# maybeLx/MVSFormerPlusPlus

Hardware: AMD Instinct MI355X
Metric: ref-views/sec at 1152x1536 N=5 D=192 4-stage; achieved HBM GB/s vs peak (higher is better)
Workload: dtype fp16 operands/storage, fp32 accumulate (every stage; 1-2 fp16 MFMA terms)

## Files before the change

mvsformerplusplus_amd/csrc/vis_kernels.hip:

```cpp
#include "mvs_common.h"

namespace mvs {

typedef __bf16 vs_bf16x8 __attribute__((ext_vector_type(8)));
typedef __bf16 vs_bf16x4 __attribute__((ext_vector_type(4)));

constexpr int VS_TW = 60;
constexpr int VS_P = 64;
constexpr int VS_RING = 4;
constexpr int VS_SH_MAX = 64;
constexpr int VS_EP = VS_P + 2;
constexpr int VS_ENT_BYTES = (VS_SH_MAX + 6) * VS_EP * 4;
constexpr int VS_F16_PLANE_SHIFT = 0;
template <bool F16>
struct VsL {
    static constexpr int POSB = F16 ? 16 : 32;
    static constexpr int PLANE = ((VS_RING * VS_P + 2) * POSB + 255) / 256 * 256 + (F16 ? VS_F16_PLANE_SHIFT : 16);
    static constexpr int LAYER = 2 * PLANE;
    static constexpr int LDS = 2 * LAYER + VS_ENT_BYTES;
};
typedef _Float16 vs_f16x8 __attribute__((ext_vector_type(8)));
typedef _Float16 vs_f16x4 __attribute__((ext_vector_type(4)));

#ifndef MVS_OPAQUE_VEC
#define MVS_OPAQUE_VEC "v"
#endif

__device__ __forceinline__ vs_f16x4 vs_mask4(vs_f16x4 h, bool in) {
    typedef unsigned vs_u32x2 __attribute__((ext_vector_type(2)));
    vs_u32x2 u = __builtin_bit_cast(vs_u32x2, h);
    u[0] = in ? u[0] : 0u;
    u[1] = in ? u[1] : 0u;
    return __builtin_bit_cast(vs_f16x4, u);
}

__device__ __forceinline__ vs_f16x4 vs_cvt4(const float* v) {
    typedef float vs_f32x4 __attribute__((ext_vector_type(4)));
    return __builtin_convertvector((vs_f32x4){v[0], v[1], v[2], v[3]}, vs_f16x4);
}

__device__ __forceinline__ void vs_split4(const float* v, vs_bf16x4& hi, vs_bf16x4& lo) {
#pragma unroll
    for (int j = 0; j < 4; ++j) {
        const __bf16 h = (__bf16)v[j];
        hi[j] = h;
        lo[j] = (__bf16)(v[j] - (float)h);
    }
}

template <int SLOT0, int POSB>
__device__ __forceinline__ int vs_step_off(int laneoff, int tapsel, int t) {
    const int tapA = 2 * t, tapB = 2 * t + 1 < 9 ? 2 * t + 1 : 8;
    const int offA = (((SLOT0 + tapA / 3) & (VS_RING - 1)) * VS_P + tapA % 3) * POSB;
    const int offB = (((SLOT0 + tapB / 3) & (VS_RING - 1)) * VS_P + tapB % 3) * POSB;
    return laneoff + (tapsel ? offB : offA);
}

struct VsOperand { vs_bf16x8 h, l; };
template <bool F16>
__device__ __forceinline__ VsOperand vs_load(const char* p) {
    VsOperand o;
    o.h = *reinterpret_cast<const vs_bf16x8*>(p);
    if constexpr (!F16) o.l = *reinterpret_cast<const vs_bf16x8*>(p + 16);
    else o.l = o.h;
    return o;
}

template <bool F16>
__device__ __forceinline__ f32x4 vs_mfma_lo(const vs_bf16x8& wl, const VsOperand& x, f32x4 a) {
    if constexpr (F16) return __builtin_amdgcn_mfma_f32_16x16x32_f16(__builtin_bit_cast(vs_f16x8, wl), __builtin_bit_cast(vs_f16x8, x.h), a, 0, 0, 0);
    else return __builtin_amdgcn_mfma_f32_16x16x32_bf16(wl, x.h, a, 0, 0, 0);
}
template <bool F16>
__device__ __forceinline__ f32x4 vs_mfma_hi(const vs_bf16x8& wh, const VsOperand& x, f32x4 a) {
    if constexpr (F16) return __builtin_amdgcn_mfma_f32_16x16x32_f16(__builtin_bit_cast(vs_f16x8, wh), __builtin_bit_cast(vs_f16x8, x.h), a, 0, 0, 0);
    else return __builtin_amdgcn_mfma_f32_16x16x32_bf16(wh, x.h, a, 0, 0, 0);
}

template <int SLOT0, bool F16, bool ONE = false>
__device__ __forceinline__ f32x4 vs_layer_row(const char* lds_layer, int laneoff, int tapsel, const vs_bf16x8* wh, const vs_bf16x8* wl, f32x4 init) {
    constexpr int POSB = VsL<F16>::POSB;
    f32x4 a0 = {0.0f, 0.0f, 0.0f, 0.0f}, a1 = a0, a2 = init;
    VsOperand cur = vs_load<F16>(lds_layer + vs_step_off<SLOT0, POSB>(laneoff, tapsel, 0));
#pragma unroll
    for (int t = 0; t < 5; ++t) {
        VsOperand nxt = cur;
        if (t < 4) nxt = vs_load<F16>(lds_layer + vs_step_off<SLOT0, POSB>(laneoff, tapsel, t + 1));
        __builtin_amdgcn_sched_barrier(0);
        if constexpr (!ONE) a0 = vs_mfma_lo<F16>(wl[t], cur, a0);
        if constexpr (!F16) a1 = __builtin_amdgcn_mfma_f32_16x16x32_bf16(wh[t], cur.l, a1, 0, 0, 0);
        a2 = vs_mfma_hi<F16>(wh[t], cur, a2);
        cur = nxt;
    }
    return a0 + a1 + a2;
}

template <int SLOT2, int SLOT3, bool F16, bool ONE = false>
__device__ __forceinline__ void vs_two_layer_rows(const char* lds1, const char* lds2, int laneoff, int tapsel, const vs_bf16x8* w2h,
                                                  const vs_bf16x8* w2l, const vs_bf16x8* w3h, const vs_bf16x8* w3l, f32x4& out2, f32x4& out3) {
    constexpr int POSB = VsL<F16>::POSB;
    f32x4 a = out2, c = out3;
    VsOperand cb = vs_load<F16>(lds1 + vs_step_off<SLOT2, POSB>(laneoff, tapsel, 0));
    VsOperand cc = vs_load<F16>(lds2 + vs_step_off<SLOT3, POSB>(laneoff, tapsel, 0));
#pragma unroll
    for (int t = 0; t < 5; ++t) {
        VsOperand nb = cb, nc = cc;
        if (t < 4) {
            nb = vs_load<F16>(lds1 + vs_step_off<SLOT2, POSB>(laneoff, tapsel, t + 1));
            nc = vs_load<F16>(lds2 + vs_step_off<SLOT3, POSB>(laneoff, tapsel, t + 1));
        }
        __builtin_amdgcn_sched_barrier(0);
        if constexpr (!ONE) {
            a = vs_mfma_lo<F16>(w2l[t], cb, a);
            c = vs_mfma_lo<F16>(w3l[t], cc, c);
        }
        if constexpr (!F16) {
            a = __builtin_amdgcn_mfma_f32_16x16x32_bf16(w2h[t], cb.l, a, 0, 0, 0);
            c = __builtin_amdgcn_mfma_f32_16x16x32_bf16(w3h[t], cc.l, c, 0, 0, 0);
        }
        a = vs_mfma_hi<F16>(w2h[t], cb, a);
        c = vs_mfma_hi<F16>(w3h[t], cc, c);
        cb = nb;
        cc = nc;
    }
    out2 = a;
    out3 = c;
}

template <int V> struct VsInt { static constexpr int value = V; };

template <bool F16, bool ONE = false>
__global__ __launch_bounds__(256) void vis_cnn_kernel(const float* __restrict__ ent, const float* __restrict__ w1 ,
                                                      const float* __restrict__ b1, const void* __restrict__ wp2, const float* __restrict__ b2,
                                                      const void* __restrict__ wp3, const float* __restrict__ b3, const float* __restrict__ w4,
                                                      const float* __restrict__ b4, float* __restrict__ vis, int H, int W, int SH) {
    HIP_DYNAMIC_SHARED(float4, lds4)
    char* lds1 = reinterpret_cast<char*>(lds4);
    constexpr int VS_POSB = VsL<F16>::POSB, VS_PLANE = VsL<F16>::PLANE, VS_LAYER = VsL<F16>::LAYER;
    char* lds2 = lds1 + VS_LAYER;
    const int tid = (int)threadIdx.x, lane = tid & 63;
    const int wave = __builtin_amdgcn_readfirstlane(tid >> 6);
    const int li = lane & 15, g = lane >> 4;
    const int x0 = (int)blockIdx.x * VS_TW, r0 = (int)blockIdx.y * SH;
    const int r1 = r0 + SH < H ? r0 + SH : H;
    const float* e = ent + (size_t)blockIdx.z * H * W;
    float* vo = vis + (size_t)blockIdx.z * H * W;

    vs_bf16x8 w2h[5], w2l[5], w3h[5], w3l[5];
    {
        const vs_bf16x8* q2 = reinterpret_cast<const vs_bf16x8*>(wp2) + lane;
        const vs_bf16x8* q3 = reinterpret_cast<const vs_bf16x8*>(wp3) + lane;
#pragma unroll
        for (int t = 0; t < 5; ++t) {
            w2h[t] = q2[(t * 2) * 64]; w2l[t] = q2[(t * 2 + 1) * 64];
            w3h[t] = q3[(t * 2) * 64]; w3l[t] = q3[(t * 2 + 1) * 64];
#ifndef MVS_NO_OPAQUE_VEC
            if constexpr (ONE) asm volatile("" : "+" MVS_OPAQUE_VEC(w2h[t]), "+" MVS_OPAQUE_VEC(w3h[t]));
            else asm volatile("" : "+" MVS_OPAQUE_VEC(w2h[t]), "+" MVS_OPAQUE_VEC(w2l[t]), "+" MVS_OPAQUE_VEC(w3h[t]), "+" MVS_OPAQUE_VEC(w3l[t]));
#endif
        }
    }
    constexpr bool L1MFMA = F16 && ONE;
    vs_f16x8 w1a = {0, 0, 0, 0, 0, 0, 0, 0};
    f32x4 b1q = {0.0f, 0.0f, 0.0f, 0.0f};
    if constexpr (L1MFMA) {
        const int kh = g < 3 ? g : 0;
#pragma unroll
        for (int kw = 0; kw < 3; ++kw) {
            const _Float16 wv = g < 3 ? (_Float16)w1[(kh * 3 + kw) * 16 + li] : (_Float16)0.0f;
            w1a[kw] = wv;
            w1a[3 + kw] = wv;
        }
#pragma unroll
        for (int r = 0; r < 4; ++r) b1q[r] = b1[4 * g + r];
    }
    float w1s[9][4], b1s[4];
#pragma unroll
    for (int t = 0; t < 9; ++t)
#pragma unroll
        for (int r = 0; r < 4; ++r) w1s[t][r] = w1[t * 16 + 4 * wave + r];
#pragma unroll
    for (int r = 0; r < 4; ++r) b1s[r] = b1[4 * wave + r];
    float b2v[4], b3v[4], w4v[4];
#pragma unroll
    for (int r = 0; r < 4; ++r) {
        b2v[r] = b2[4 * g + r];
        b3v[r] = g < 2 ? b3[4 * g + r] : 0.0f;
        w4v[r] = g < 2 ? w4[4 * g + r] : 0.0f;
    }
    const float bias4 = b4[0];

    const int xa = x0 - 2 + lane;
    const int i0 = r0 - 2, i1 = r1 + 4;
    float* ent_s = reinterpret_cast<float*>(lds1 + 2 * VS_LAYER);
    {
        const int nrow = r1 - r0 + 6;
        for (int idx = tid; idx < nrow * VS_EP; idx += 256) {
            const int rr = idx / VS_EP, cc = idx - rr * VS_EP;
            const int yy = r0 - 3 + rr, xx = x0 - 3 + cc;
            ent_s[idx] = (yy >= 0 && yy < H && xx >= 0 && xx < W) ? e[(size_t)yy * W + xx] : 0.0f;
        }
    }
    __syncthreads();
    const int colmaskA = xa >= 0 && xa < W;
    const int wrA = (wave >> 1) * VS_PLANE + lane * VS_POSB + (wave & 1) * 8;
    const int laneoff = (g & 1) * VS_PLANE + (16 * wave + li) * VS_POSB;
    const int wrB = (g >> 1) * VS_PLANE + (16 * wave + li) * VS_POSB + (g & 1) * 8;
    const int tapsel = g >> 1;
    const int c2 = 16 * wave + li;
    const int xb = x0 - 1 + c2, xc = x0 + c2;

    auto iteration = [&](auto phase, auto steady, int i) __attribute__((always_inline)) {
        constexpr int PH = decltype(phase)::value;
        constexpr bool STEADY = decltype(steady)::value != 0;
        if constexpr (L1MFMA) {
            if (STEADY || i <= r1 + 1) {
                const float* ep = ent_s + (i - 1 + (g < 3 ? g : 2) - (r0 - 3)) * VS_EP + c2;
                const float e0 = ep[0], e1 = ep[1], e2 = ep[2];
                typedef float vs_f32x2 __attribute__((ext_vector_type(2)));
                typedef _Float16 vs_f16x2 __attribute__((ext_vector_type(2)));
                typedef unsigned vs_u32x4 __attribute__((ext_vector_type(4)));
                const unsigned p0 = __builtin_bit_cast(unsigned, __builtin_convertvector((vs_f32x2){e0, e1}, vs_f16x2));
                const float l0 = MVS_FMA_MIX_LO(p0, -1.0f, e0), l1 = MVS_FMA_MIX_HI(p0, -1.0f, e1);
                const unsigned p1 = __builtin_bit_cast(unsigned, __builtin_convertvector((vs_f32x2){e2, l0}, vs_f16x2));
                const float l2 = MVS_FMA_MIX_LO(p1, -1.0f, e2);
                const unsigned p2 = __builtin_bit_cast(unsigned, __builtin_convertvector((vs_f32x2){l1, l2}, vs_f16x2));
                const vs_f16x8 bop = __builtin_bit_cast(vs_f16x8, (vs_u32x4){p0, p1, p2, 0u});
                const f32x4 r1v = __builtin_amdgcn_mfma_f32_16x16x32_f16(w1a, bop, b1q, 0, 0, 0);
                const int xa1 = x0 - 2 + c2;
                const bool in = xa1 >= 0 && xa1 < W && i >= 0 && i < H;
                float a[4];
#pragma unroll
                for (int r = 0; r < 4; ++r) a[r] = fmaxf(r1v[r], 0.0f);
                *reinterpret_cast<vs_f16x4*>(lds1 + wrB + PH * (VS_P * VS_POSB)) = vs_mask4(vs_cvt4(a), in);
            }
        } else if (STEADY || i <= r1 + 1) {
            float er[3][3];
            const float* ep = ent_s + (i - 1 - (r0 - 3)) * VS_EP + lane;
#pragma unroll
            for (int kh = 0; kh < 3; ++kh)
#pragma unroll
                for (int kw = 0; kw < 3; ++kw) er[kh][kw] = ep[kh * VS_EP + kw];
            typedef float f32x2 __attribute__((ext_vector_type(2)));
            f32x2 a01 = {b1s[0], b1s[1]}, a23 = {b1s[2], b1s[3]};
#pragma unroll
            for (int kh = 0; kh < 3; ++kh)
#pragma unroll
                for (int kw = 0; kw < 3; ++kw) {
                    const f32x2 ev = {er[kh][kw], er[kh][kw]};
                    a01 = __builtin_elementwise_fma(ev, (f32x2){w1s[kh * 3 + kw][0], w1s[kh * 3 + kw][1]}, a01);
                    a23 = __builtin_elementwise_fma(ev, (f32x2){w1s[kh * 3 + kw][2], w1s[kh * 3 + kw][3]}, a23);
                }
            float a[4] = {a01[0], a01[1], a23[0], a23[1]};
            const bool in = colmaskA && i >= 0 && i < H;
#pragma unroll
            for (int r = 0; r < 4; ++r) a[r] = F16 ? fmaxf(a[r], 0.0f) : (in ? fmaxf(a[r], 0.0f) : 0.0f);
            char* p = lds1 + wrA + PH * (VS_P * VS_POSB);
            if constexpr (F16) {
                *reinterpret_cast<vs_f16x4*>(p) = vs_mask4(vs_cvt4(a), in);
            } else {
                vs_bf16x4 hi, lo;
                vs_split4(a, hi, lo);
                *reinterpret_cast<vs_bf16x4*>(p) = hi;
                *reinterpret_cast<vs_bf16x4*>(p + 16) = lo;
            }
        }
        const int yb = i - 2, yc = i - 4;
        const bool doB = STEADY || (yb >= r0 - 1 && yb <= r1), doC = STEADY || yc >= r0;
        constexpr int S2 = (PH + 1) & 3, S3 = (PH + 3) & 3;
        f32x4 acc2 = {b2v[0], b2v[1], b2v[2], b2v[3]}, acc3 = {b3v[0], b3v[1], b3v[2], b3v[3]};
        if (STEADY || (doB && doC)) vs_two_layer_rows<S2, S3, F16, ONE>(lds1, lds2, laneoff, tapsel, w2h, w2l, w3h, w3l, acc2, acc3);
        else if (doB) acc2 = vs_layer_row<S2, F16, ONE>(lds1, laneoff, tapsel, w2h, w2l, acc2);
        else if (doC) acc3 = vs_layer_row<S3, F16, ONE>(lds2, laneoff, tapsel, w3h, w3l, acc3);
        if (doB) {
            const bool in = xb >= 0 && xb < W && yb >= 0 && yb < H;
            float v[4];
#pragma unroll
            for (int r = 0; r < 4; ++r) v[r] = F16 ? fmaxf(acc2[r], 0.0f) : (in ? fmaxf(acc2[r], 0.0f) : 0.0f);
            char* p = lds2 + wrB + ((PH + 2) & 3) * (VS_P * VS_POSB);
            if constexpr (F16) {
                *reinterpret_cast<vs_f16x4*>(p) = vs_mask4(vs_cvt4(v), in);
            } else {
                vs_bf16x4 hi, lo;
                vs_split4(v, hi, lo);
                *reinterpret_cast<vs_bf16x4*>(p) = hi;
                *reinterpret_cast<vs_bf16x4*>(p + 16) = lo;
            }
        }
        if (doC) {
            float part = 0.0f;
#pragma unroll
            for (int r = 0; r < 4; ++r) part += fmaxf(acc3[r], 0.0f) * w4v[r];
            part += __shfl_xor(part, 16);
            if (g == 0 && c2 < VS_TW && xc < W && yc < r1) {
                const float z = part + bias4;
                vo[(size_t)yc * W + xc] = __builtin_amdgcn_rcpf(1.0f + __builtin_amdgcn_exp2f(-z * 1.4426950408889634f));
            }
        }
        __syncthreads();
    };
    auto general = [&](int i) __attribute__((always_inline)) {
        switch (i & 3) {
            case 0: iteration(VsInt<0>(), VsInt<0>(), i); break;
            case 1: iteration(VsInt<1>(), VsInt<0>(), i); break;
            case 2: iteration(VsInt<2>(), VsInt<0>(), i); break;
            default: iteration(VsInt<3>(), VsInt<0>(), i); break;
        }
    };
    int i = i0;
    for (; i < i1 && (i < r0 + 4 || (i & 3) != 0); ++i) general(i);
    for (; i + 3 <= r1 + 1; i += 4) {
        iteration(VsInt<0>(), VsInt<1>(), i);
        iteration(VsInt<1>(), VsInt<1>(), i + 1);
        iteration(VsInt<2>(), VsInt<1>(), i + 2);
        iteration(VsInt<3>(), VsInt<1>(), i + 3);
    }
    for (; i < i1; ++i) general(i);
}


template <bool F16, bool ONE = false>
static int vis_weight_stream_t(const float* entropy, const float* w1, const float* b1, const void* w2, const float* b2, const void* w3,
                               const float* b3, const float* w4, const float* b4, float* vis, int N, int H, int W, hipStream_t st) {
    constexpr int VS_LDS = VsL<F16>::LDS;
    const int strips = (int)ceil_div(W, VS_TW);
    const long long per_seg = (long long)strips * N, resident = (160 * 1024 / VS_LDS < 4 ? 160 * 1024 / VS_LDS : 4) * 256;
    int segs = (int)ceil_div(H, VS_SH_MAX), SH = (int)ceil_div(H, segs);
    long long best = -1;
    for (int sg = (int)ceil_div(H, VS_SH_MAX); sg <= (H + 7) / 8; ++sg) {
        const int sh = (int)ceil_div(H, sg);
        const long long rounds = (per_seg * ceil_div(H, sh) + resident - 1) / resident;
        const long long cost = rounds * (sh + 6);
        if (best < 0 || cost < best) { best = cost; segs = (int)ceil_div(H, sh); SH = sh; }
    }
    if (VS_LDS > 48 * 1024)
        hipFuncSetAttribute(reinterpret_cast<const void*>(&vis_cnn_kernel<F16, ONE>), hipFuncAttributeMaxDynamicSharedMemorySize, VS_LDS);
    hipLaunchKernelGGL((vis_cnn_kernel<F16, ONE>), dim3(strips, segs, N), dim3(256), VS_LDS, st, entropy, w1, b1, w2, b2, w3, b3, w4, b4, vis, H, W, SH);
    return check_launch("vis_cnn_kernel");
}

int vis_weight_stream_bf16x3(const float* entropy, const float* w1, const float* b1, const void* w2, const float* b2, const void* w3,
                             const float* b3, const float* w4, const float* b4, float* vis, int N, int H, int W, hipStream_t st, int f16) {
    if (f16 == 2) return vis_weight_stream_t<true, true>(entropy, w1, b1, w2, b2, w3, b3, w4, b4, vis, N, H, W, st);
    return f16 ? vis_weight_stream_t<true>(entropy, w1, b1, w2, b2, w3, b3, w4, b4, vis, N, H, W, st)
               : vis_weight_stream_t<false>(entropy, w1, b1, w2, b2, w3, b3, w4, b4, vis, N, H, W, st);
}

}
```

Before: 683.4.

## Add row-pair visibility CNN kernel computing two output rows per layer-3 pass

Adds a new fused visibility CNN kernel with a 6-slot ring that computes the final conv layer for two output rows at once. It packs layer-3 weights so a single MFMA chain covers both rows, and interleaves that chain with the layer-2 MFMAs, with explicit register prefetch of LDS operands. The goal is to cut per-row layer-3 work and synchronisation and to improve MFMA issue density. The new path is enabled by default for the f16==2 mode, with an env var to fall back. It uses more LDS per block, capped at four blocks per CU, and needs even segment heights, which adds complexity and edge-handling risk.

```diff
diff --git a/mvsformerplusplus_amd/csrc/vis_kernels.hip b/mvsformerplusplus_amd/csrc/vis_kernels.hip
--- a/mvsformerplusplus_amd/csrc/vis_kernels.hip
+++ b/mvsformerplusplus_amd/csrc/vis_kernels.hip
@@ -1,4 +1,6 @@
 #include "mvs_common.h"
+
+#include <cstdlib>
 
 namespace mvs {
 
@@ -319,6 +321,243 @@
 }
 
 
+constexpr int VP_RING = 6;
+constexpr int VP_SH_MAX = 48;
+constexpr int VP_POSB = 16;
+constexpr int VP_SLOT = VS_P * VP_POSB;
+constexpr int VP_PLANE = ((VP_RING * VS_P + 2) * VP_POSB + 255) / 256 * 256;
+constexpr int VP_LAYER = 2 * VP_PLANE;
+constexpr int VP_LDS = 2 * VP_LAYER + (VP_SH_MAX + 6) * VS_EP * 4;
+static_assert(VP_LDS <= 40 * 1024, "four resident blocks per CU");
+
+template <int SLOT0, int NTAP>
+__device__ __forceinline__ int vp_step_off(int laneoff, int tapsel, int t) {
+    const int tapA = 2 * t, tapB = 2 * t + 1 < NTAP ? 2 * t + 1 : NTAP - 1;
+    const int offA = (((SLOT0 + tapA / 3) % VP_RING) * VS_P + tapA % 3) * VP_POSB;
+    const int offB = (((SLOT0 + tapB / 3) % VP_RING) * VS_P + tapB % 3) * VP_POSB;
+    return laneoff + (tapsel ? offB : offA);
+}
+
+__device__ __forceinline__ f32x4 vp_mfma(const vs_f16x8& w, const vs_f16x8& x, f32x4 a) {
+    return __builtin_amdgcn_mfma_f32_16x16x32_f16(w, x, a, 0, 0, 0);
+}
+
+template <int SLOT0, int NTAP, int NSTEP>
+__device__ __forceinline__ f32x4 vp_layer_row(const char* lds_layer, int laneoff, int tapsel, const vs_f16x8* w, f32x4 init) {
+    f32x4 a = init;
+    vs_f16x8 cur = *reinterpret_cast<const vs_f16x8*>(lds_layer + vp_step_off<SLOT0, NTAP>(laneoff, tapsel, 0));
+#pragma unroll
+    for (int t = 0; t < NSTEP; ++t) {
+        vs_f16x8 nxt = cur;
+        if (t + 1 < NSTEP) nxt = *reinterpret_cast<const vs_f16x8*>(lds_layer + vp_step_off<SLOT0, NTAP>(laneoff, tapsel, t + 1));
+        __builtin_amdgcn_sched_barrier(0);
+        a = vp_mfma(w[t], cur, a);
+        cur = nxt;
+    }
+    return a;
+}
+
+template <int SLOT2, int SLOT3>
+__device__ __forceinline__ void vp_two_layer_rows(const char* lds1, const char* lds2, int laneoff, int tapsel, const vs_f16x8* w2, const vs_f16x8* w3p,
+                                                  f32x4& out2, f32x4& out3) {
+    f32x4 a = out2, c = out3;
+    vs_f16x8 cb = *reinterpret_cast<const vs_f16x8*>(lds1 + vp_step_off<SLOT2, 9>(laneoff, tapsel, 0));
+    vs_f16x8 cc = *reinterpret_cast<const vs_f16x8*>(lds2 + vp_step_off<SLOT3, 12>(laneoff, tapsel, 0));
+#pragma unroll
+    for (int t = 0; t < 6; ++t) {
+        vs_f16x8 nb = cb, nc = cc;
+        if (t < 4) nb = *reinterpret_cast<const vs_f16x8*>(lds1 + vp_step_off<SLOT2, 9>(laneoff, tapsel, t + 1));
+        if (t < 5) nc = *reinterpret_cast<const vs_f16x8*>(lds2 + vp_step_off<SLOT3, 12>(laneoff, tapsel, t + 1));
+        __builtin_amdgcn_sched_barrier(0);
+        if (t < 5) a = vp_mfma(w2[t], cb, a);
+        c = vp_mfma(w3p[t], cc, c);
+        cb = nb;
+        cc = nc;
+    }
+    out2 = a;
+    out3 = c;
+}
+
+__global__ __launch_bounds__(256, 4) void vis_cnn_pairs_kernel(const float* __restrict__ ent, const float* __restrict__ w1 ,
+                                                            const float* __restrict__ b1, const void* __restrict__ wp2, const float* __restrict__ b2,
+                                                            const void* __restrict__ wp3, const float* __restrict__ b3, const float* __restrict__ w4,
+                                                            const float* __restrict__ b4, float* __restrict__ vis, int H, int W, int SH) {
+    HIP_DYNAMIC_SHARED(float4, lds4)
+    char* lds1 = reinterpret_cast<char*>(lds4);
+    char* lds2 = lds1 + VP_LAYER;
+    const int tid = (int)threadIdx.x, lane = tid & 63;
+    const int wave = __builtin_amdgcn_readfirstlane(tid >> 6);
+    const int li = lane & 15, g = lane >> 4;
+    const int x0 = (int)blockIdx.x * VS_TW, r0 = (int)blockIdx.y * SH;
+    const int r1 = r0 + SH < H ? r0 + SH : H;
+    const float* e = ent + (size_t)blockIdx.z * H * W;
+    float* vo = vis + (size_t)blockIdx.z * H * W;
+
+    vs_f16x8 w2[5], w3p[6];
+    {
+        const vs_f16x8* q2 = reinterpret_cast<const vs_f16x8*>(wp2) + lane;
+        const vs_f16x8* q3 = reinterpret_cast<const vs_f16x8*>(wp3);
+#pragma unroll
+        for (int t = 0; t < 5; ++t) w2[t] = q2[(t * 2) * 64];
+#pragma unroll
+        for (int s = 0; s < 6; ++s) {
+            const int w = 2 * s + (g >> 1), tap = li < 8 ? w : w - 3;
+            const bool valid = tap >= 0 && tap < 9;
+            const int tc = valid ? tap : 0;
+            const vs_f16x8 f = q3[((tc >> 1) * 2) * 64 + ((tc & 1) * 2 + (g & 1)) * 16 + (li & 7)];
+            const vs_f16x8 zero = {0, 0, 0, 0, 0, 0, 0, 0};
+            w3p[s] = valid ? f : zero;
+        }
+#ifndef MVS_NO_OPAQUE_VEC
+#pragma unroll
+        for (int t = 0; t < 5; ++t) asm volatile("" : "+" MVS_OPAQUE_VEC(w2[t]));
+#pragma unroll
+        for (int s = 0; s < 6; ++s) asm volatile("" : "+" MVS_OPAQUE_VEC(w3p[s]));
+#endif
+    }
+    vs_f16x8 w1a = {0, 0, 0, 0, 0, 0, 0, 0};
+    f32x4 b1q = {0.0f, 0.0f, 0.0f, 0.0f};
+    {
+        const int kh = g < 3 ? g : 0;
+#pragma unroll
+        for (int kw = 0; kw < 3; ++kw) {
+            const _Float16 wv = g < 3 ? (_Float16)w1[(kh * 3 + kw) * 16 + li] : (_Float16)0.0f;
+            w1a[kw] = wv;
+            w1a[3 + kw] = wv;
+        }
+#pragma unroll
+        for (int r = 0; r < 4; ++r) b1q[r] = b1[4 * g + r];
+    }
+    float b2v[4], b3v[4], w4s[8];
+#pragma unroll
+    for (int r = 0; r < 4; ++r) {
+        b2v[r] = b2[4 * g + r];
+        b3v[r] = b3[4 * (g & 1) + r];
+    }
+#pragma unroll
+    for (int k = 0; k < 8; ++k) w4s[k] = w4[k];
+    const float bias4 = b4[0];
+
+    const int i0 = r0 - 2, i1 = r1 + 4 + (r1 & 1);
+    float* ent_s = reinterpret_cast<float*>(lds1 + 2 * VP_LAYER);
+    {
+        const int nrow = r1 - r0 + 6;
+        for (int idx = tid; idx < nrow * VS_EP; idx += 256) {
+            const int rr = idx / VS_EP, cc = idx - rr * VS_EP;
+            const int yy = r0 - 3 + rr, xx = x0 - 3 + cc;
+            ent_s[idx] = (yy >= 0 && yy < H && xx >= 0 && xx < W) ? e[(size_t)yy * W + xx] : 0.0f;
+        }
+        if (r1 & 1)
+            for (int idx = tid; idx < VP_LAYER / 16; idx += 256) reinterpret_cast<float4*>(lds2)[idx] = make_float4(0.0f, 0.0f, 0.0f, 0.0f);
+    }
+    __syncthreads();
+    const int laneoff = (g & 1) * VP_PLANE + (16 * wave + li) * VP_POSB;
+    const int wrB = (g >> 1) * VP_PLANE + (16 * wave + li) * VP_POSB + (g & 1) * 8;
+    const int tapsel = g >> 1;
+    const int c2 = 16 * wave + li;
+    const int xa1 = x0 - 2 + c2, xb = x0 - 1 + c2, xc = x0 + c2;
+
+    auto iteration = [&](auto phase, auto steady, int i) __attribute__((always_inline)) {
+        constexpr int PH = decltype(phase)::value;
+        constexpr bool STEADY = decltype(steady)::value != 0;
+        constexpr bool PAIR = (PH & 1) != 0;
+        if (STEADY || i <= r1 + 1) {
+            const float* ep = ent_s + (i - 1 + (g < 3 ? g : 2) - (r0 - 3)) * VS_EP + c2;
+            const float e0 = ep[0], e1 = ep[1], e2 = ep[2];
+            typedef float vs_f32x2 __attribute__((ext_vector_type(2)));
+            typedef _Float16 vs_f16x2 __attribute__((ext_vector_type(2)));
+            typedef unsigned vs_u32x4 __attribute__((ext_vector_type(4)));
+            const unsigned p0 = __builtin_bit_cast(unsigned, __builtin_convertvector((vs_f32x2){e0, e1}, vs_f16x2));
+            const float l0 = MVS_FMA_MIX_LO(p0, -1.0f, e0), l1 = MVS_FMA_MIX_HI(p0, -1.0f, e1);
+            const unsigned p1 = __builtin_bit_cast(unsigned, __builtin_convertvector((vs_f32x2){e2, l0}, vs_f16x2));
+            const float l2 = MVS_FMA_MIX_LO(p1, -1.0f, e2);
+            const unsigned p2 = __builtin_bit_cast(unsigned, __builtin_convertvector((vs_f32x2){l1, l2}, vs_f16x2));
+            const vs_f16x8 bop = __builtin_bit_cast(vs_f16x8, (vs_u32x4){p0, p1, p2, 0u});
+            const f32x4 r1v = vp_mfma(w1a, bop, b1q);
+            const bool in = xa1 >= 0 && xa1 < W && i >= 0 && i < H;
+            float a[4];
+#pragma unroll
+            for (int r = 0; r < 4; ++r) a[r] = fmaxf(r1v[r], 0.0f);
+            *reinterpret_cast<vs_f16x4*>(lds1 + wrB + PH * VP_SLOT) = vs_mask4(vs_cvt4(a), in);
+        }
+        const int yb = i - 2, yc = i - 5;
+        const bool doB = STEADY || (yb >= r0 - 1 && yb <= r1), doC = PAIR && (STEADY || (yc >= r0 && yc < r1));
+        constexpr int S2 = (PH + 3) % VP_RING, S3 = PH;
+        f32x4 acc2 = {b2v[0], b2v[1], b2v[2], b2v[3]}, acc3 = {b3v[0], b3v[1], b3v[2], b3v[3]};
+        if constexpr (PAIR) {
+            if (STEADY || (doB && doC)) vp_two_layer_rows<S2, S3>(lds1, lds2, laneoff, tapsel, w2, w3p, acc2, acc3);
+            else if (doB) acc2 = vp_layer_row<S2, 9, 5>(lds1, laneoff, tapsel, w2, acc2);
+            else if (doC) acc3 = vp_layer_row<S3, 12, 6>(lds2, laneoff, tapsel, w3p, acc3);
+        } else {
+            if (doB) acc2 = vp_layer_row<S2, 9, 5>(lds1, laneoff, tapsel, w2, acc2);
+        }
+        if (doB) {
+            const bool in = xb >= 0 && xb < W && yb >= 0 && yb < H;
+            float v[4];
+#pragma unroll
+            for (int r = 0; r < 4; ++r) v[r] = fmaxf(acc2[r], 0.0f);
+            *reinterpret_cast<vs_f16x4*>(lds2 + wrB + ((PH + 4) % VP_RING) * VP_SLOT) = vs_mask4(vs_cvt4(v), in);
+        }
+        if constexpr (PAIR) {
+            if (doC) {
+                float p0 = 0.0f, p1 = 0.0f;
+#pragma unroll
+                for (int r = 0; r < 4; ++r) {
+                    const float v = fmaxf(acc3[r], 0.0f);
+                    p0 += v * w4s[r];
+                    p1 += v * w4s[4 + r];
+                }
+                float part = (g & 1) ? p1 : p0;
+                part += __shfl_xor(part, 16);
+                const int yo = yc + (g >> 1);
+                if ((g & 1) == 0 && c2 < VS_TW && xc < W && yo < r1) {
+                    const float z = part + bias4;
+                    vo[(size_t)yo * W + xc] = __builtin_amdgcn_rcpf(1.0f + __builtin_amdgcn_exp2f(-z * 1.4426950408889634f));
+                }
+            }
+        }
+        __syncthreads();
+    };
+    auto general = [&](int i) __attribute__((always_inline)) {
+        switch ((i + VP_RING) % VP_RING) {
+            case 0: iteration(VsInt<0>(), VsInt<0>(), i); break;
+            case 1: iteration(VsInt<1>(), VsInt<0>(), i); break;
+            case 2: iteration(VsInt<2>(), VsInt<0>(), i); break;
+            case 3: iteration(VsInt<3>(), VsInt<0>(), i); break;
+            case 4: iteration(VsInt<4>(), VsInt<0>(), i); break;
+            default: iteration(VsInt<5>(), VsInt<0>(), i); break;
+        }
+    };
+    int i = i0;
+    for (; i < i1 && (i < r0 + 5 || (i + VP_RING) % VP_RING != 0); ++i) general(i);
+    for (; i + 5 <= r1 + 1; i += 6) {
+        iteration(VsInt<0>(), VsInt<1>(), i);
+        iteration(VsInt<1>(), VsInt<1>(), i + 1);
+        iteration(VsInt<2>(), VsInt<1>(), i + 2);
+        iteration(VsInt<3>(), VsInt<1>(), i + 3);
+        iteration(VsInt<4>(), VsInt<1>(), i + 4);
+        iteration(VsInt<5>(), VsInt<1>(), i + 5);
+    }
+    for (; i < i1; ++i) general(i);
+}
+
+static int vis_weight_stream_pairs(const float* entropy, const float* w1, const float* b1, const void* w2, const float* b2, const void* w3,
+                                   const float* b3, const float* w4, const float* b4, float* vis, int N, int H, int W, hipStream_t st) {
+    const int strips = (int)ceil_div(W, VS_TW);
+    const long long per_seg = (long long)strips * N, resident = 4 * 256;
+    int segs = 0, SH = 0;
+    long long best = -1;
+    for (int sg = (int)ceil_div(H, VP_SH_MAX); sg <= (H + 7) / 8; ++sg) {
+        int sh = (int)ceil_div(H, sg);
+        sh += sh & 1;
+        const long long rounds = (per_seg * ceil_div(H, sh) + resident - 1) / resident;
+        const long long cost = rounds * (sh + 6);
+        if (best < 0 || cost < best) { best = cost; segs = (int)ceil_div(H, sh); SH = sh; }
+    }
+    hipLaunchKernelGGL(vis_cnn_pairs_kernel, dim3(strips, segs, N), dim3(256), VP_LDS, st, entropy, w1, b1, w2, b2, w3, b3, w4, b4, vis, H, W, SH);
+    return check_launch("vis_cnn_pairs_kernel");
+}
+
 template <bool F16, bool ONE = false>
 static int vis_weight_stream_t(const float* entropy, const float* w1, const float* b1, const void* w2, const float* b2, const void* w3,
                                const float* b3, const float* w4, const float* b4, float* vis, int N, int H, int W, hipStream_t st) {
@@ -341,7 +580,12 @@
 
 int vis_weight_stream_bf16x3(const float* entropy, const float* w1, const float* b1, const void* w2, const float* b2, const void* w3,
                              const float* b3, const float* w4, const float* b4, float* vis, int N, int H, int W, hipStream_t st, int f16) {
-    if (f16 == 2) return vis_weight_stream_t<true, true>(entropy, w1, b1, w2, b2, w3, b3, w4, b4, vis, N, H, W, st);
+    if (f16 == 2) {
+        const char* sw = getenv("MVS_VIS_ROW_PAIRS");
+        const bool pairs = (sw == nullptr || sw[0] == '\0') ? true : sw[0] != '0';
+        if (pairs) return vis_weight_stream_pairs(entropy, w1, b1, w2, b2, w3, b3, w4, b4, vis, N, H, W, st);
+        return vis_weight_stream_t<true, true>(entropy, w1, b1, w2, b2, w3, b3, w4, b4, vis, N, H, W, st);
+    }
     return f16 ? vis_weight_stream_t<true>(entropy, w1, b1, w2, b2, w3, b3, w4, b4, vis, N, H, W, st)
                : vis_weight_stream_t<false>(entropy, w1, b1, w2, b2, w3, b3, w4, b4, vis, N, H, W, st);
 }
```

Result: no change. 683.6 (median of 6 runs) (+0.0%).
